# aclike/dynamic_multiview_3d

Measured on AMD Instinct MI355X. Metric: train images/sec, appearance-flow encoder-decoder 128x128x3 (fwd+bwd+Adam), higher is better.
Workload: dtype bf16x3; 1 GPU; appflow_offset: AppearanceFlowModel 128x128x3, batch 64 per GPU, Adam lr 1e-4, random-init weights (reference initialisers); global_batch=64, parallelism=dp1

## Files before the change

### dynamic_multiview_3d_amd/csrc/fc.hip

```cpp
#include "conv_common.h"
#include <algorithm>

namespace mv3d {

struct FcParams {
    const float* X;
    const float* W;
    float* Part;
    int M, R, N, x_ld;
    int w_ld;
    int nsplit, chunks_total;
};

template <bool TRANS, int MT>
__global__ __launch_bounds__(256) void fc_stream_kernel(const FcParams p) {
    constexpr int LDA = 33;
    constexpr int ROWS = 32 * MT;
    __shared__ float As[2][ROWS * LDA];
    const int tid = threadIdx.x;
    const int lane = tid & 63, wave = tid >> 6;
    const int li = lane & 31, lh = lane >> 5;
    const int n0 = blockIdx.x * 128 + wave * 32;
    const int ks = blockIdx.y;
    const int c_begin = (int)((int64_t)p.chunks_total * ks / p.nsplit);
    const int c_end = (int)((int64_t)p.chunks_total * (ks + 1) / p.nsplit);

    f32x16 acc[MT];
#pragma unroll
    for (int m = 0; m < MT; ++m)
#pragma unroll
        for (int r = 0; r < 16; ++r) acc[m][r] = 0.f;

    const int col = n0 + li;
    const int colc = col < p.N ? col : p.N - 1;

    constexpr int A_PASSES = ROWS / 32;
    float4 ra[A_PASSES];
    auto load_a = [&](int chunk) {
        const int r0 = chunk * 32 + (tid & 7) * 4;
        const bool k_ok = r0 + 4 <= p.R;
#pragma unroll
        for (int ps = 0; ps < A_PASSES; ++ps) {
            const int row = ps * 32 + (tid >> 3);
            const bool ok = k_ok && row < p.M;
            const float4 v = *reinterpret_cast<const float4*>(p.X + (int64_t)(ok ? row : 0) * p.x_ld + (ok ? r0 : 0));
            ra[ps] = ok ? v : make_float4(0.f, 0.f, 0.f, 0.f);
        }
    };
    auto store_a = [&](int buf) {
#pragma unroll
        for (int ps = 0; ps < A_PASSES; ++ps) {
            float* d = &As[buf][(ps * 32 + (tid >> 3)) * LDA + (tid & 7) * 4];
            d[0] = ra[ps].x; d[1] = ra[ps].y; d[2] = ra[ps].z; d[3] = ra[ps].w;
        }
    };
    float b0[16], b1[16];
    auto load_b = [&](float (&b)[16], int chunk) {
        const int r0 = chunk * 32 + lh * 16;
        const int rc = (r0 + 16 <= p.R) ? r0 : 0;
        if constexpr (TRANS) {
            const float4* src = reinterpret_cast<const float4*>(p.W + (int64_t)colc * p.w_ld + rc);
#pragma unroll
            for (int j = 0; j < 4; ++j) {
                const float4 v = src[j];
                b[4 * j] = v.x; b[4 * j + 1] = v.y; b[4 * j + 2] = v.z; b[4 * j + 3] = v.w;
            }
        } else {
            const float* src = p.W + (int64_t)rc * p.w_ld + colc;
#pragma unroll
            for (int kp = 0; kp < 16; ++kp) { b[kp] = *src; src += p.w_ld; }
        }
    };

    if (c_begin < c_end) {
        load_a(c_begin);
        load_b(b1, c_begin);
        store_a(0);
        __syncthreads();
        int buf = 0;
        for (int c = c_begin; c < c_end; ++c, buf ^= 1) {
            const bool more = c + 1 < c_end;
#pragma unroll
            for (int kp = 0; kp < 16; ++kp) b0[kp] = b1[kp];
            if (more) { load_a(c + 1); load_b(b1, c + 1); }
            const float* ap = &As[buf][li * LDA + lh * 16];
#pragma unroll
            for (int kp = 0; kp < 16; ++kp)
#pragma unroll
                for (int m = 0; m < MT; ++m)
                    acc[m] = __builtin_amdgcn_mfma_f32_32x32x2f32(ap[m * 32 * LDA + kp], b0[kp], acc[m], 0, 0, 0);
            if (more) store_a(buf ^ 1);
            __syncthreads();
        }
    }
#pragma unroll
    for (int m = 0; m < MT; ++m)
#pragma unroll
        for (int r = 0; r < 16; ++r) {
            const int row = m * 32 + (r & 3) + 8 * (r >> 2) + 4 * lh;
            if (row < p.M && col < p.N) p.Part[((int64_t)ks * p.M + row) * p.N + col] = acc[m][r];
        }
}


typedef __bf16 fbf16x8 __attribute__((ext_vector_type(8)));
typedef __bf16 fbf16x4 __attribute__((ext_vector_type(4)));
typedef short fs16x4 __attribute__((ext_vector_type(4)));

__device__ __forceinline__ void fsplit4(float a, float b, float c, float d, uint2& hi, uint2& lo) {
    fbf16x4 h, l;
    h[0] = (__bf16)a; h[1] = (__bf16)b; h[2] = (__bf16)c; h[3] = (__bf16)d;
    l[0] = (__bf16)(a - (float)h[0]); l[1] = (__bf16)(b - (float)h[1]);
    l[2] = (__bf16)(c - (float)h[2]); l[3] = (__bf16)(d - (float)h[3]);
    hi = __builtin_bit_cast(uint2, h);
    lo = __builtin_bit_cast(uint2, l);
}

template <bool TRANS, int MT>
__global__ __launch_bounds__(256) void fc_stream_b3_kernel(const FcParams p) {
    constexpr int ROWS = 32 * MT;
    constexpr int RSB = 80;
    __shared__ __attribute__((aligned(16))) unsigned char As[2][2][ROWS * RSB];
    const int tid = threadIdx.x;
    const int lane = tid & 63, wave = tid >> 6;
    const int li = lane & 31, lh = lane >> 5;
    const int n0 = blockIdx.x * 128 + wave * 32;
    const int ks = blockIdx.y;
    const int c_begin = (int)((int64_t)p.chunks_total * ks / p.nsplit);
    const int c_end = (int)((int64_t)p.chunks_total * (ks + 1) / p.nsplit);

    f32x16 acc[MT];
#pragma unroll
    for (int m = 0; m < MT; ++m)
#pragma unroll
        for (int r = 0; r < 16; ++r) acc[m][r] = 0.f;

    const int col = n0 + li;
    const int colc = col < p.N ? col : p.N - 1;

    constexpr int A_PASSES = ROWS / 32;
    constexpr int RING = MT <= 2 ? 6 : 4;
    float4 rq[RING][A_PASSES];
    auto load_a = [&](float4 (&ra)[A_PASSES], int chunk) {
        const int r0 = chunk * 32 + (tid & 7) * 4;
        const bool k_ok = r0 + 4 <= p.R;
#pragma unroll
        for (int ps = 0; ps < A_PASSES; ++ps) {
            const int row = ps * 32 + (tid >> 3);
            const bool ok = k_ok && row < p.M;
            const float4 v = *reinterpret_cast<const float4*>(p.X + (int64_t)(ok ? row : 0) * p.x_ld + (ok ? r0 : 0));
            ra[ps] = ok ? v : make_float4(0.f, 0.f, 0.f, 0.f);
        }
    };
    auto store_a = [&](const float4 (&ra)[A_PASSES], int buf) {
#pragma unroll
        for (int ps = 0; ps < A_PASSES; ++ps) {
            uint2 hi, lo;
            fsplit4(ra[ps].x, ra[ps].y, ra[ps].z, ra[ps].w, hi, lo);
            const int off = (ps * 32 + (tid >> 3)) * RSB + (tid & 7) * 8;
            *reinterpret_cast<uint2*>(&As[buf][0][off]) = hi;
            *reinterpret_cast<uint2*>(&As[buf][1][off]) = lo;
        }
    };
    float bq[RING][16];
    auto load_b = [&](float (&b)[16], int chunk) {
        const int r0 = chunk * 32 + lh * 16;
        const int rc = (r0 + 16 <= p.R) ? r0 : 0;
        if constexpr (TRANS) {
            const float4* src = reinterpret_cast<const float4*>(p.W + (int64_t)colc * p.w_ld + rc);
#pragma unroll
            for (int j = 0; j < 4; ++j) {
                const float4 v = src[j];
                b[4 * j] = v.x; b[4 * j + 1] = v.y; b[4 * j + 2] = v.z; b[4 * j + 3] = v.w;
            }
        } else {
            const float* src = p.W + (int64_t)rc * p.w_ld + colc;
#pragma unroll
            for (int kp = 0; kp < 16; ++kp) { b[kp] = *src; src += p.w_ld; }
        }
    };
    auto mma = [&](const float (&b)[16], int buf) {
#pragma unroll
        for (int s2 = 0; s2 < 2; ++s2) {
            uint2 h0, l0, h1, l1;
            fsplit4(b[8 * s2], b[8 * s2 + 1], b[8 * s2 + 2], b[8 * s2 + 3], h0, l0);
            fsplit4(b[8 * s2 + 4], b[8 * s2 + 5], b[8 * s2 + 6], b[8 * s2 + 7], h1, l1);
            const fbf16x8 bh = __builtin_bit_cast(fbf16x8, make_uint4(h0.x, h0.y, h1.x, h1.y));
            const fbf16x8 bl = __builtin_bit_cast(fbf16x8, make_uint4(l0.x, l0.y, l1.x, l1.y));
#pragma unroll
            for (int m = 0; m < MT; ++m) {
                const int off = (m * 32 + li) * RSB + (lh * 16 + 8 * s2) * 2;
                const fbf16x8 ah = __builtin_bit_cast(fbf16x8, *reinterpret_cast<const uint4*>(&As[buf][0][off]));
                const fbf16x8 al = __builtin_bit_cast(fbf16x8, *reinterpret_cast<const uint4*>(&As[buf][1][off]));
                acc[m] = __builtin_amdgcn_mfma_f32_32x32x16_bf16(al, bh, acc[m], 0, 0, 0);
                acc[m] = __builtin_amdgcn_mfma_f32_32x32x16_bf16(ah, bl, acc[m], 0, 0, 0);
                acc[m] = __builtin_amdgcn_mfma_f32_32x32x16_bf16(ah, bh, acc[m], 0, 0, 0);
            }
        }
    };

    if (c_begin < c_end) {
#pragma unroll
        for (int u = 0; u < RING - 1; ++u) {
            const int cu = c_begin + u < c_end ? c_begin + u : c_end - 1;
            load_a(rq[u], cu);
            load_b(bq[u], cu);
        }
        store_a(rq[0], 0);
        __syncthreads();
        int buf = 0;
        constexpr int NCH = 16;
        if (c_end - c_begin == NCH) {
#pragma unroll
            for (int i = 0; i < NCH; ++i) {
                if (i + RING - 1 < NCH) {
                    load_a(rq[(i + RING - 1) % RING], c_begin + i + RING - 1);
                    load_b(bq[(i + RING - 1) % RING], c_begin + i + RING - 1);
                }
                __builtin_amdgcn_sched_barrier(0);
                mma(bq[i % RING], i & 1);
                if (i + 1 < NCH) store_a(rq[(i + 1) % RING], (i + 1) & 1);
                __syncthreads();
            }
        } else
        for (int c = c_begin; c < c_end; c += RING) {
#pragma unroll
            for (int u = 0; u < RING; ++u) {
                const int cc = c + u;
                if (cc < c_end) {
                    const int cn = cc + RING - 1 < c_end ? cc + RING - 1 : c_end - 1;
                    load_a(rq[(u + RING - 1) % RING], cn);
                    load_b(bq[(u + RING - 1) % RING], cn);
                    mma(bq[u], buf);
                    if (cc + 1 < c_end) store_a(rq[(u + 1) % RING], buf ^ 1);
                    __syncthreads();
                    buf ^= 1;
                }
            }
        }
    }
#pragma unroll
    for (int m = 0; m < MT; ++m)
#pragma unroll
        for (int r = 0; r < 16; ++r) {
            const int row = m * 32 + (r & 3) + 8 * (r >> 2) + 4 * lh;
            if (row < p.M && col < p.N) p.Part[((int64_t)ks * p.M + row) * p.N + col] = acc[m][r];
        }
}

struct FcWgradParams {
    const float* X; const float* DY; float* dW; float* db;
    int B, C, K, x_ld, dy_ld;
    int ktiles;
    float* M1; float* V2;
    const float* state;
};

__device__ __forceinline__ void adam_elem(float g, float& pv, float& mv, float& vv, float alpha, float omb1, float omb2, float eps) {
#pragma clang fp contract(off)
    mv += (g - mv) * omb1;
    vv += (g * g - vv) * omb2;
    pv -= (mv * alpha) / (sqrtf(vv) + eps);
}

__global__ __launch_bounds__(256) void fc_wgrad_kernel(const FcWgradParams p) {
    __shared__ __attribute__((aligned(16))) float xs[64 * 128];
    __shared__ __attribute__((aligned(16))) float dys[64 * 128];
    const int tid = threadIdx.x;
    const int lane = tid & 63, wave = tid >> 6;
    const int li = lane & 31, lh = lane >> 5;
    const int kt = blockIdx.x % p.ktiles, ct = blockIdx.x / p.ktiles;
    const int c0 = ct * 128, k0 = kt * 128;
    const int ws = wave >> 1, wt = wave & 1;
    f32x16 acc[2][2];
#pragma unroll
    for (int a = 0; a < 2; ++a)
#pragma unroll
        for (int b = 0; b < 2; ++b)
#pragma unroll
            for (int r = 0; r < 16; ++r) acc[a][b][r] = 0.f;
    float sb[2] = {0.f, 0.f};
    for (int b0 = 0; b0 < p.B; b0 += 64) {
        if (b0) __syncthreads();
        float4 vx[8], vy[8];
#pragma unroll
        for (int j = 0; j < 8; ++j) {
            const int row = b0 + (tid >> 5) + 8 * j;
            const int cx = c0 + (tid & 31) * 4, ky = k0 + (tid & 31) * 4;
            const bool okx = row < p.B && cx + 4 <= p.C, oky = row < p.B && ky + 4 <= p.K;
            const float4 tx = *reinterpret_cast<const float4*>(p.X + (okx ? (int64_t)row * p.x_ld + cx : 0));
            const float4 ty = *reinterpret_cast<const float4*>(p.DY + (oky ? (int64_t)row * p.dy_ld + ky : 0));
            vx[j] = okx ? tx : make_float4(0.f, 0.f, 0.f, 0.f);
            vy[j] = oky ? ty : make_float4(0.f, 0.f, 0.f, 0.f);
        }
#pragma unroll
        for (int j = 0; j < 8; ++j) {
            const int r = (tid >> 5) + 8 * j;
            *reinterpret_cast<float4*>(&xs[r * 128 + (tid & 31) * 4]) = vx[j];
            *reinterpret_cast<float4*>(&dys[r * 128 + (tid & 31) * 4]) = vy[j];
        }
        __syncthreads();
        const float* pa = xs + lh * 128 + ws * 64 + li;
        const float* pb = dys + lh * 128 + wt * 64 + li;
#pragma unroll 4
        for (int bp = 0; bp < 32; ++bp) {
            const float a0 = pa[bp * 256], a1 = pa[bp * 256 + 32];
            const float q0 = pb[bp * 256], q1 = pb[bp * 256 + 32];
            acc[0][0] = __builtin_amdgcn_mfma_f32_32x32x2f32(a0, q0, acc[0][0], 0, 0, 0);
            acc[0][1] = __builtin_amdgcn_mfma_f32_32x32x2f32(a0, q1, acc[0][1], 0, 0, 0);
            acc[1][0] = __builtin_amdgcn_mfma_f32_32x32x2f32(a1, q0, acc[1][0], 0, 0, 0);
            acc[1][1] = __builtin_amdgcn_mfma_f32_32x32x2f32(a1, q1, acc[1][1], 0, 0, 0);
            sb[0] += q0; sb[1] += q1;
        }
    }
#pragma unroll
    for (int s = 0; s < 2; ++s)
#pragma unroll
        for (int t = 0; t < 2; ++t) {
            const int k = k0 + wt * 64 + t * 32 + li;
#pragma unroll
            for (int r = 0; r < 16; ++r) {
                const int c = c0 + ws * 64 + s * 32 + (r & 3) + 8 * (r >> 2) + 4 * lh;
                if (c < p.C && k < p.K) p.dW[(int64_t)c * p.K + k] = acc[s][t][r];
            }
        }
    if (p.db && ct == 0 && ws == 0) {
#pragma unroll
        for (int t = 0; t < 2; ++t) {
            const float v = sb[t] + __shfl_xor(sb[t], 32);
            const int k = k0 + wt * 64 + t * 32 + li;
            if (lh == 0 && k < p.K) p.db[k] = v;
        }
    }
}


__device__ __forceinline__ uint2 ftr_read(const unsigned char* lds_ptr) {
    fs16x4 v = __builtin_amdgcn_ds_read_tr16_b64_v4i16((__attribute__((address_space(3))) fs16x4*)lds_ptr);
    return __builtin_bit_cast(uint2, v);
}

template <int OPT>
__global__ __launch_bounds__(256) void fc_wgrad_b3_kernel(const FcWgradParams p) {
    constexpr int RS = 320;
    __shared__ __attribute__((aligned(16))) unsigned char xs[2][32 * RS];
    __shared__ __attribute__((aligned(16))) unsigned char dys[2][32 * RS];
    __shared__ float bred[8][128];
    const int tid = threadIdx.x;
    const int lane = tid & 63, wave = tid >> 6;
    const int li = lane & 31, lh = lane >> 5;
    const int kt = blockIdx.x % p.ktiles, ct = blockIdx.x / p.ktiles;
    const int c0 = ct * 128, k0 = kt * 128;
    const int ws = wave >> 1, wt = wave & 1;
    const int g16 = (lane >> 4) & 1, q = (lane >> 2) & 3, pp = lane & 3;
    f32x16 acc[2][2];
#pragma unroll
    for (int a = 0; a < 2; ++a)
#pragma unroll
        for (int b = 0; b < 2; ++b)
#pragma unroll
            for (int r = 0; r < 16; ++r) acc[a][b][r] = 0.f;
    float4 bs = make_float4(0.f, 0.f, 0.f, 0.f);
    for (int b0 = 0; b0 < p.B; b0 += 32) {
        if (b0) __syncthreads();
        float4 vx[4], vy[4];
#pragma unroll
        for (int j = 0; j < 4; ++j) {
            const int row = b0 + (tid >> 5) + 8 * j;
            const int cx = c0 + (tid & 31) * 4, ky = k0 + (tid & 31) * 4;
            const bool okx = row < p.B && cx + 4 <= p.C, oky = row < p.B && ky + 4 <= p.K;
            const float4 tx = *reinterpret_cast<const float4*>(p.X + (okx ? (int64_t)row * p.x_ld + cx : 0));
            const float4 ty = *reinterpret_cast<const float4*>(p.DY + (oky ? (int64_t)row * p.dy_ld + ky : 0));
            vx[j] = okx ? tx : make_float4(0.f, 0.f, 0.f, 0.f);
            vy[j] = oky ? ty : make_float4(0.f, 0.f, 0.f, 0.f);
        }
#pragma unroll
        for (int j = 0; j < 4; ++j) {
            const int off = ((tid >> 5) + 8 * j) * RS + (tid & 31) * 8;
            uint2 hi, lo;
            fsplit4(vx[j].x, vx[j].y, vx[j].z, vx[j].w, hi, lo);
            *reinterpret_cast<uint2*>(&xs[0][off]) = hi;
            *reinterpret_cast<uint2*>(&xs[1][off]) = lo;
            fsplit4(vy[j].x, vy[j].y, vy[j].z, vy[j].w, hi, lo);
            *reinterpret_cast<uint2*>(&dys[0][off]) = hi;
            *reinterpret_cast<uint2*>(&dys[1][off]) = lo;
            bs.x += vy[j].x; bs.y += vy[j].y; bs.z += vy[j].z; bs.w += vy[j].w;
        }
        __syncthreads();
#pragma unroll
        for (int s2 = 0; s2 < 2; ++s2) {
            const int row0 = 16 * s2 + 8 * lh + q;
            const int ra0 = row0 * RS + (16 * g16 + 4 * pp) * 2, ra1 = ra0 + 4 * RS;
            fbf16x8 ah[2], al[2], bh[2], bl[2];
#pragma unroll
            for (int t = 0; t < 2; ++t) {
                const int ca = (ws * 64 + t * 32) * 2, cb = (wt * 64 + t * 32) * 2;
                uint2 u0 = ftr_read(&xs[0][ra0 + ca]), u1 = ftr_read(&xs[0][ra1 + ca]);
                ah[t] = __builtin_bit_cast(fbf16x8, make_uint4(u0.x, u0.y, u1.x, u1.y));
                u0 = ftr_read(&xs[1][ra0 + ca]); u1 = ftr_read(&xs[1][ra1 + ca]);
                al[t] = __builtin_bit_cast(fbf16x8, make_uint4(u0.x, u0.y, u1.x, u1.y));
                u0 = ftr_read(&dys[0][ra0 + cb]); u1 = ftr_read(&dys[0][ra1 + cb]);
                bh[t] = __builtin_bit_cast(fbf16x8, make_uint4(u0.x, u0.y, u1.x, u1.y));
                u0 = ftr_read(&dys[1][ra0 + cb]); u1 = ftr_read(&dys[1][ra1 + cb]);
                bl[t] = __builtin_bit_cast(fbf16x8, make_uint4(u0.x, u0.y, u1.x, u1.y));
            }
#pragma unroll
            for (int a = 0; a < 2; ++a)
#pragma unroll
                for (int b = 0; b < 2; ++b) {
                    acc[a][b] = __builtin_amdgcn_mfma_f32_32x32x16_bf16(al[a], bh[b], acc[a][b], 0, 0, 0);
                    acc[a][b] = __builtin_amdgcn_mfma_f32_32x32x16_bf16(ah[a], bl[b], acc[a][b], 0, 0, 0);
                    acc[a][b] = __builtin_amdgcn_mfma_f32_32x32x16_bf16(ah[a], bh[b], acc[a][b], 0, 0, 0);
                }
        }
    }
    float alpha = 0.f, omb1 = 0.f, omb2 = 0.f, eps = 0.f, gscale = 1.f;
    float lr = 0.f, mu = 0.f;
    bool nesterov = false;
    if constexpr (OPT == OPT_MOMENTUM || OPT == OPT_GD) {
        lr = p.state[MV3D_SGD_LR]; mu = p.state[MV3D_SGD_MOMENTUM]; nesterov = p.state[MV3D_SGD_NESTEROV] != 0.f;
        gscale = p.state[MV3D_SGD_GSCALE];
    }
    if constexpr (OPT == OPT_ADAM) {
        const float lr = p.state[0], b1 = p.state[1], b2 = p.state[2], b1p = p.state[4], b2p = p.state[5];
        eps = p.state[3]; gscale = p.state[6];
        {
#pragma clang fp contract(off)
            alpha = lr * sqrtf(1.0f - b2p) / (1.0f - b1p);
            omb1 = 1.0f - b1; omb2 = 1.0f - b2;
        }
    }
#pragma unroll
    for (int s = 0; s < 2; ++s)
#pragma unroll
        for (int t = 0; t < 2; ++t) {
            const int k = k0 + wt * 64 + t * 32 + li;
            if constexpr (OPT == OPT_ADAM) {
                {
                    float pv[16], mv[16], vv[16];
#pragma unroll
                    for (int r = 0; r < 16; ++r) {
                        const int c = c0 + ws * 64 + s * 32 + (r & 3) + 8 * (r >> 2) + 4 * lh;
                        const int64_t idx = (c < p.C && k < p.K) ? (int64_t)c * p.K + k : 0;
                        pv[r] = p.dW[idx]; mv[r] = p.M1[idx]; vv[r] = p.V2[idx];
                    }
#pragma unroll
                    for (int r = 0; r < 16; ++r) adam_elem(acc[s][t][r] * gscale, pv[r], mv[r], vv[r], alpha, omb1, omb2, eps);
#pragma unroll
                    for (int r = 0; r < 16; ++r) {
                        const int c = c0 + ws * 64 + s * 32 + (r & 3) + 8 * (r >> 2) + 4 * lh;
                        if (c < p.C && k < p.K) {
                            const int64_t idx = (int64_t)c * p.K + k;
                            p.dW[idx] = pv[r]; p.M1[idx] = mv[r]; p.V2[idx] = vv[r];
                        }
                    }
                }
            } else if constexpr (OPT == OPT_MOMENTUM || OPT == OPT_GD) {
                float pv[16], av[16];
#pragma unroll
                for (int r = 0; r < 16; ++r) {
                    const int c = c0 + ws * 64 + s * 32 + (r & 3) + 8 * (r >> 2) + 4 * lh;
                    const int64_t idx = (c < p.C && k < p.K) ? (int64_t)c * p.K + k : 0;
                    pv[r] = p.dW[idx];
                    if constexpr (OPT == OPT_MOMENTUM) av[r] = p.M1[idx];
                }
#pragma unroll
                for (int r = 0; r < 16; ++r) {
                    if constexpr (OPT == OPT_MOMENTUM) momentum_elem(acc[s][t][r] * gscale, pv[r], av[r], lr, mu, nesterov);
                    else gd_elem(acc[s][t][r] * gscale, pv[r], lr);
                }
#pragma unroll
                for (int r = 0; r < 16; ++r) {
                    const int c = c0 + ws * 64 + s * 32 + (r & 3) + 8 * (r >> 2) + 4 * lh;
                    if (c < p.C && k < p.K) {
                        const int64_t idx = (int64_t)c * p.K + k;
                        p.dW[idx] = pv[r];
                        if constexpr (OPT == OPT_MOMENTUM) p.M1[idx] = av[r];
                    }
                }
            } else {
#pragma unroll
                for (int r = 0; r < 16; ++r) {
                    const int c = c0 + ws * 64 + s * 32 + (r & 3) + 8 * (r >> 2) + 4 * lh;
                    if (c < p.C && k < p.K) p.dW[(int64_t)c * p.K + k] = acc[s][t][r];
                }
            }
        }
    if (p.db && ct == 0) {
        float* br = &bred[tid >> 5][(tid & 31) * 4];
        br[0] = bs.x; br[1] = bs.y; br[2] = bs.z; br[3] = bs.w;
        __syncthreads();
        if (tid < 128) {
            float t = 0.f;
#pragma unroll
            for (int r = 0; r < 8; ++r) t += bred[r][tid];
            if (k0 + tid < p.K) p.db[k0 + tid] = t;
        }
    }
}

static bool fc_stream_ok(int B, int in, int out, const void* x, int x_ld, const void* W, bool trans) {
    if (B < 1 || B > 128) return false;
    const int R = trans ? out : in;
    if (R < 256 || R % 16 != 0 || x_ld % 4 != 0) return false;
    if ((reinterpret_cast<uintptr_t>(x) & 15) || (reinterpret_cast<uintptr_t>(W) & 15)) return false;
    if (trans && (out % 4 != 0)) return false;
    return !(disabled_paths() & 16);
}

static int fc_target_wgs() {
    static int v = -1;
    if (v < 0) { const char* e = getenv("MV3D_FC_WGS"); v = e ? atoi(e) : 256; }
    return v;
}

size_t fc_stream_ws_bytes(int B, int in, int out, bool trans) {
    const int R = trans ? out : in, N = trans ? in : out;
    const int chunks = cdiv(R, 32);
    int nsplit = std::max(1, std::min(chunks / 4, cdiv(fc_target_wgs(), cdiv(N, 128))));
    return (size_t)nsplit * B * N * sizeof(float);
}

int try_fc_stream(bool trans, int B, int in, int out, const void* x, int x_ld, const void* W, void* y, int y_ld,
                  const mv3d_epilogue* epi, void* ws, size_t wsb, void* stream, const char* who,
                  void (*fill_epi)(IgemmParams&, const mv3d_epilogue*), void (*launch_epi)(const IgemmParams&, int, hipStream_t)) {
    if (!fc_stream_ok(B, in, out, x, x_ld, W, trans)) return 1;
    FcParams p = {};
    p.X = (const float*)x; p.W = (const float*)W; p.Part = (float*)ws;
    p.M = B; p.R = trans ? out : in; p.N = trans ? in : out; p.x_ld = x_ld; p.w_ld = out;
    p.chunks_total = cdiv(p.R, 32);
    p.nsplit = std::max(1, std::min(p.chunks_total / 4, cdiv(fc_target_wgs(), cdiv(p.N, 128))));
    const size_t need = (size_t)p.nsplit * B * p.N * sizeof(float);
    if (!ws || wsb < need) return 1;
    dim3 grid(cdiv(p.N, 128), p.nsplit);
    const int MT = cdiv(B, 32);
    const double flops = 2.0 * B * (double)in * out, bytes = 4.0 * ((double)in * out + (double)B * (in + out));
    const bool b3 = !(disabled_paths() & 4096);
    int rc = dispatch(stream, OpInfo{b3 ? (trans ? "fc_stream_b3<dgrad>" : "fc_stream_b3<fwd>") : (trans ? "fc_stream<dgrad>" : "fc_stream<fwd>"), flops, bytes}, [=](hipStream_t s) {
        if (b3) {
            if (trans) {
                if (MT <= 1) fc_stream_b3_kernel<true, 1><<<grid, 256, 0, s>>>(p);
                else if (MT == 2) fc_stream_b3_kernel<true, 2><<<grid, 256, 0, s>>>(p);
                else fc_stream_b3_kernel<true, 4><<<grid, 256, 0, s>>>(p);
            } else {
                if (MT <= 1) fc_stream_b3_kernel<false, 1><<<grid, 256, 0, s>>>(p);
                else if (MT == 2) fc_stream_b3_kernel<false, 2><<<grid, 256, 0, s>>>(p);
                else fc_stream_b3_kernel<false, 4><<<grid, 256, 0, s>>>(p);
            }
        } else if (trans) {
            if (MT <= 1) fc_stream_kernel<true, 1><<<grid, 256, 0, s>>>(p);
            else if (MT == 2) fc_stream_kernel<true, 2><<<grid, 256, 0, s>>>(p);
            else fc_stream_kernel<true, 4><<<grid, 256, 0, s>>>(p);
        } else {
            if (MT <= 1) fc_stream_kernel<false, 1><<<grid, 256, 0, s>>>(p);
            else if (MT == 2) fc_stream_kernel<false, 2><<<grid, 256, 0, s>>>(p);
            else fc_stream_kernel<false, 4><<<grid, 256, 0, s>>>(p);
        }
        return launched(who);
    });
    if (rc != MV3D_OK) return rc;
    IgemmParams e = {};
    e.N = 1; e.Hc = 1; e.Wc = B; e.Cc = p.N; e.c_ld = y_ld; e.Out = (float*)y; e.Part = (float*)ws; e.ksplit = p.nsplit;
    fill_epi(e, epi);
    const int64_t total = (int64_t)B * p.N;
    const int blocks = (int)std::min<int64_t>(cdiv64(total, 256), 4096);
    return dispatch(stream, OpInfo{"fc_splitk_epilogue", 0.0, (double)total * 4.0 * (p.nsplit + 1)}, [=](hipStream_t s) {
        launch_epi(e, blocks, s);
        return launched("igemm_splitk_epilogue");
    });
}

int try_fc_wgrad(int B, int in, int out, const void* x, int x_ld, const void* dy, int dy_ld, void* dM, void* db, void* stream, const char* who) {
    if (B < 2 || in < 64 || out < 64 || (disabled_paths() & 16)) return 1;
    if (in % 4 || out % 4 || x_ld % 4 || dy_ld % 4 || (reinterpret_cast<uintptr_t>(x) & 15) || (reinterpret_cast<uintptr_t>(dy) & 15)) return 1;
    FcWgradParams p = {(const float*)x, (const float*)dy, (float*)dM, (float*)db, B, in, out, x_ld, dy_ld, cdiv(out, 128), nullptr, nullptr, nullptr};
    const int items = cdiv(in, 128) * p.ktiles;
    const double flops = 2.0 * B * (double)in * out, bytes = 4.0 * ((double)in * out + (double)B * (in + out));
    const bool b3 = !(disabled_paths() & 4096);
    return dispatch(stream, OpInfo{b3 ? "fc_wgrad_b3" : "fc_wgrad", flops, bytes}, [=](hipStream_t s) {
        if (b3) fc_wgrad_b3_kernel<OPT_NONE><<<items, 256, 0, s>>>(p);
        else fc_wgrad_kernel<<<items, 256, 0, s>>>(p);
        return launched(who);
    });
}

int try_fc_wgrad_adam(int B, int in, int out, const void* x, int x_ld, const void* dy, int dy_ld, void* P, void* M1, void* V2, void* db,
                      const void* state, void* stream, const char* who) {
    if (B < 2 || in < 64 || out < 64 || (disabled_paths() & (16 | 4096))) return 1;
    if (in % 4 || out % 4 || x_ld % 4 || dy_ld % 4 || (reinterpret_cast<uintptr_t>(x) & 15) || (reinterpret_cast<uintptr_t>(dy) & 15)) return 1;
    FcWgradParams p = {(const float*)x, (const float*)dy, (float*)P, (float*)db, B, in, out, x_ld, dy_ld, cdiv(out, 128), (float*)M1, (float*)V2, (const float*)state};
    const int items = cdiv(in, 128) * p.ktiles;
    const double flops = 2.0 * B * (double)in * out, bytes = 24.0 * (double)in * out + 4.0 * (double)B * (in + out);
    return dispatch(stream, OpInfo{"fc_wgrad_adam_b3", flops, bytes}, [=](hipStream_t s) {
        fc_wgrad_b3_kernel<OPT_ADAM><<<items, 256, 0, s>>>(p);
        return launched(who);
    });
}

int try_fc_wgrad_sgd(int B, int in, int out, const void* x, int x_ld, const void* dy, int dy_ld, void* P, void* A, void* db,
                     const void* state, void* stream, const char* who) {
    if (B < 2 || in < 64 || out < 64 || (disabled_paths() & (16 | 4096))) return 1;
    if (in % 4 || out % 4 || x_ld % 4 || dy_ld % 4 || (reinterpret_cast<uintptr_t>(x) & 15) || (reinterpret_cast<uintptr_t>(dy) & 15)) return 1;
    FcWgradParams p = {(const float*)x, (const float*)dy, (float*)P, (float*)db, B, in, out, x_ld, dy_ld, cdiv(out, 128), (float*)A, nullptr, (const float*)state};
    const int items = cdiv(in, 128) * p.ktiles;
    const bool mom = A != nullptr;
    const double flops = 2.0 * B * (double)in * out, bytes = (mom ? 16.0 : 8.0) * (double)in * out + 4.0 * (double)B * (in + out);
    return dispatch(stream, OpInfo{mom ? "fc_wgrad_momentum_b3" : "fc_wgrad_sgd_b3", flops, bytes}, [=](hipStream_t s) {
        if (mom) fc_wgrad_b3_kernel<OPT_MOMENTUM><<<items, 256, 0, s>>>(p);
        else fc_wgrad_b3_kernel<OPT_GD><<<items, 256, 0, s>>>(p);
        return launched(who);
    });
}

}
```

Baseline: 38850 images/sec.

## Use buffer loads and a fully unrolled chunked pipeline in bf16x3 FC kernel

Replaces the FC streaming kernel's global pointer loads with AMD buffer-resource loads. Out-of-range rows and chunks now return zero through the hardware bounds check, so the selects and 64-bit address arithmetic go away. The old split between an unrolled 16-chunk path and a generic ring loop becomes a single 18-chunk compile-time-unrolled pipeline that early-exits on partial groups. The ring depth is fixed at 4 for all MT, where MT≤2 previously used 6. The aim is lower address and branch overhead and full unrolling for any split size, at the cost of a shallower prefetch for small batches and a new 2GB size guard.

Result: no change. 39220 images/sec, median of 6 (+0.9%).

```diff
diff --git a/dynamic_multiview_3d_amd/csrc/fc.hip b/dynamic_multiview_3d_amd/csrc/fc.hip
--- a/dynamic_multiview_3d_amd/csrc/fc.hip
+++ b/dynamic_multiview_3d_amd/csrc/fc.hip
@@ -1,5 +1,6 @@
 #include "conv_common.h"
 #include <algorithm>
+#include <utility>
 
 namespace mv3d {
 
@@ -10,6 +11,7 @@
     int M, R, N, x_ld;
     int w_ld;
     int nsplit, chunks_total;
+    int x_bytes, w_bytes;
 };
 
 template <bool TRANS, int MT>
@@ -116,10 +118,15 @@
     lo = __builtin_bit_cast(uint2, l);
 }
 
-template <bool TRANS, int MT>
+template <class F, int... Is>
+__device__ __forceinline__ void fc_chain(F& f, std::integer_sequence<int, Is...>) { (void)(f(std::integral_constant<int, Is>{}) && ...); }
+
+template <bool TRANS, int MT, int RING>
 __global__ __launch_bounds__(256) void fc_stream_b3_kernel(const FcParams p) {
     constexpr int ROWS = 32 * MT;
     constexpr int RSB = 80;
+    constexpr int NCH = 18;
+    constexpr unsigned OOR = 0x7ffffff0u;
     __shared__ __attribute__((aligned(16))) unsigned char As[2][2][ROWS * RSB];
     const int tid = threadIdx.x;
     const int lane = tid & 63, wave = tid >> 6;
@@ -137,20 +144,22 @@
 
     const int col = n0 + li;
     const int colc = col < p.N ? col : p.N - 1;
+    const __amdgpu_buffer_rsrc_t xr = __builtin_amdgcn_make_buffer_rsrc(const_cast<float*>(p.X), 0, p.x_bytes, 0x00020000);
+    const __amdgpu_buffer_rsrc_t wr = __builtin_amdgcn_make_buffer_rsrc(const_cast<float*>(p.W), 0, p.w_bytes, 0x00020000);
 
     constexpr int A_PASSES = ROWS / 32;
-    constexpr int RING = MT <= 2 ? 6 : 4;
+    unsigned va[A_PASSES];
+#pragma unroll
+    for (int ps = 0; ps < A_PASSES; ++ps) {
+        const int row = ps * 32 + (tid >> 3);
+        va[ps] = row < p.M ? ((unsigned)row * (unsigned)p.x_ld + (tid & 7) * 4) * 4u : OOR;
+    }
     float4 rq[RING][A_PASSES];
-    auto load_a = [&](float4 (&ra)[A_PASSES], int chunk) {
-        const int r0 = chunk * 32 + (tid & 7) * 4;
-        const bool k_ok = r0 + 4 <= p.R;
-#pragma unroll
-        for (int ps = 0; ps < A_PASSES; ++ps) {
-            const int row = ps * 32 + (tid >> 3);
-            const bool ok = k_ok && row < p.M;
-            const float4 v = *reinterpret_cast<const float4*>(p.X + (int64_t)(ok ? row : 0) * p.x_ld + (ok ? r0 : 0));
-            ra[ps] = ok ? v : make_float4(0.f, 0.f, 0.f, 0.f);
-        }
+    auto load_a = [&](float4 (&ra)[A_PASSES], int chunk, bool valid) {
+        const bool ok = valid && chunk * 32 + (tid & 7) * 4 + 4 <= p.R;
+#pragma unroll
+        for (int ps = 0; ps < A_PASSES; ++ps)
+            ra[ps] = __builtin_bit_cast(float4, __builtin_amdgcn_raw_buffer_load_b128(xr, ok ? va[ps] : OOR, chunk * 128, 0));
     };
     auto store_a = [&](const float4 (&ra)[A_PASSES], int buf) {
 #pragma unroll
@@ -162,21 +171,21 @@
             *reinterpret_cast<uint2*>(&As[buf][1][off]) = lo;
         }
     };
+    const unsigned vb = TRANS ? ((unsigned)colc * (unsigned)p.w_ld + lh * 16) * 4u : ((unsigned)(lh * 16) * (unsigned)p.w_ld + colc) * 4u;
     float bq[RING][16];
-    auto load_b = [&](float (&b)[16], int chunk) {
-        const int r0 = chunk * 32 + lh * 16;
-        const int rc = (r0 + 16 <= p.R) ? r0 : 0;
+    auto load_b = [&](float (&b)[16], int chunk, bool valid) {
+        const bool ok = valid && chunk * 32 + lh * 16 + 16 <= p.R;
+        const unsigned v = ok ? vb : OOR;
         if constexpr (TRANS) {
-            const float4* src = reinterpret_cast<const float4*>(p.W + (int64_t)colc * p.w_ld + rc);
 #pragma unroll
             for (int j = 0; j < 4; ++j) {
-                const float4 v = src[j];
-                b[4 * j] = v.x; b[4 * j + 1] = v.y; b[4 * j + 2] = v.z; b[4 * j + 3] = v.w;
+                const float4 t = __builtin_bit_cast(float4, __builtin_amdgcn_raw_buffer_load_b128(wr, v + 16 * j, chunk * 128, 0));
+                b[4 * j] = t.x; b[4 * j + 1] = t.y; b[4 * j + 2] = t.z; b[4 * j + 3] = t.w;
             }
         } else {
-            const float* src = p.W + (int64_t)rc * p.w_ld + colc;
-#pragma unroll
-            for (int kp = 0; kp < 16; ++kp) { b[kp] = *src; src += p.w_ld; }
+#pragma unroll
+            for (int kp = 0; kp < 16; ++kp)
+                b[kp] = __uint_as_float(__builtin_amdgcn_raw_buffer_load_b32(wr, v, (chunk * 32 + kp) * p.w_ld * 4, 0));
         }
     };
     auto mma = [&](const float (&b)[16], int buf) {
@@ -199,45 +208,29 @@
         }
     };
 
-    if (c_begin < c_end) {
+    for (int c0 = c_begin; c0 < c_end; c0 += NCH) {
+        const int n = c_end - c0 < NCH ? c_end - c0 : NCH;
 #pragma unroll
         for (int u = 0; u < RING - 1; ++u) {
-            const int cu = c_begin + u < c_end ? c_begin + u : c_end - 1;
-            load_a(rq[u], cu);
-            load_b(bq[u], cu);
+            load_a(rq[u], c0 + u, u < n);
+            load_b(bq[u], c0 + u, u < n);
         }
         store_a(rq[0], 0);
         __syncthreads();
-        int buf = 0;
-        constexpr int NCH = 16;
-        if (c_end - c_begin == NCH) {
-#pragma unroll
-            for (int i = 0; i < NCH; ++i) {
-                if (i + RING - 1 < NCH) {
-                    load_a(rq[(i + RING - 1) % RING], c_begin + i + RING - 1);
-                    load_b(bq[(i + RING - 1) % RING], c_begin + i + RING - 1);
-                }
-                __builtin_amdgcn_sched_barrier(0);
-                mma(bq[i % RING], i & 1);
-                if (i + 1 < NCH) store_a(rq[(i + 1) % RING], (i + 1) & 1);
-                __syncthreads();
-            }
-        } else
-        for (int c = c_begin; c < c_end; c += RING) {
-#pragma unroll
-            for (int u = 0; u < RING; ++u) {
-                const int cc = c + u;
-                if (cc < c_end) {
-                    const int cn = cc + RING - 1 < c_end ? cc + RING - 1 : c_end - 1;
-                    load_a(rq[(u + RING - 1) % RING], cn);
-                    load_b(bq[(u + RING - 1) % RING], cn);
-                    mma(bq[u], buf);
-                    if (cc + 1 < c_end) store_a(rq[(u + 1) % RING], buf ^ 1);
-                    __syncthreads();
-                    buf ^= 1;
-                }
-            }
-        }
+        auto step = [&](auto ic) {
+            constexpr int i = decltype(ic)::value;
+            if (i >= n) return false;
+            if constexpr (i + RING - 1 < NCH) {
+                load_a(rq[(i + RING - 1) % RING], c0 + i + RING - 1, i + RING - 1 < n);
+                load_b(bq[(i + RING - 1) % RING], c0 + i + RING - 1, i + RING - 1 < n);
+            }
+            __builtin_amdgcn_sched_barrier(0);
+            mma(bq[i % RING], i & 1);
+            if constexpr (i + 1 < NCH) store_a(rq[(i + 1) % RING], (i + 1) & 1);
+            __syncthreads();
+            return true;
+        };
+        fc_chain(step, std::make_integer_sequence<int, NCH>{});
     }
 #pragma unroll
     for (int m = 0; m < MT; ++m)
@@ -499,12 +492,14 @@
     }
 }
 
+constexpr int FC_RING = 4;
 static bool fc_stream_ok(int B, int in, int out, const void* x, int x_ld, const void* W, bool trans) {
     if (B < 1 || B > 128) return false;
     const int R = trans ? out : in;
     if (R < 256 || R % 16 != 0 || x_ld % 4 != 0) return false;
     if ((reinterpret_cast<uintptr_t>(x) & 15) || (reinterpret_cast<uintptr_t>(W) & 15)) return false;
     if (trans && (out % 4 != 0)) return false;
+    if ((int64_t)in * out * 4 >= 0x7ffffff0 || ((int64_t)(B - 1) * x_ld + R) * 4 >= 0x7ffffff0) return false;
     return !(disabled_paths() & 16);
 }
 
@@ -528,6 +523,7 @@
     FcParams p = {};
     p.X = (const float*)x; p.W = (const float*)W; p.Part = (float*)ws;
     p.M = B; p.R = trans ? out : in; p.N = trans ? in : out; p.x_ld = x_ld; p.w_ld = out;
+    p.x_bytes = (int)(((int64_t)(B - 1) * x_ld + p.R) * 4); p.w_bytes = (int)((int64_t)in * out * 4);
     p.chunks_total = cdiv(p.R, 32);
     p.nsplit = std::max(1, std::min(p.chunks_total / 4, cdiv(fc_target_wgs(), cdiv(p.N, 128))));
     const size_t need = (size_t)p.nsplit * B * p.N * sizeof(float);
@@ -539,13 +535,13 @@
     int rc = dispatch(stream, OpInfo{b3 ? (trans ? "fc_stream_b3<dgrad>" : "fc_stream_b3<fwd>") : (trans ? "fc_stream<dgrad>" : "fc_stream<fwd>"), flops, bytes}, [=](hipStream_t s) {
         if (b3) {
             if (trans) {
-                if (MT <= 1) fc_stream_b3_kernel<true, 1><<<grid, 256, 0, s>>>(p);
-                else if (MT == 2) fc_stream_b3_kernel<true, 2><<<grid, 256, 0, s>>>(p);
-                else fc_stream_b3_kernel<true, 4><<<grid, 256, 0, s>>>(p);
+                if (MT <= 1) fc_stream_b3_kernel<true, 1, FC_RING><<<grid, 256, 0, s>>>(p);
+                else if (MT == 2) fc_stream_b3_kernel<true, 2, FC_RING><<<grid, 256, 0, s>>>(p);
+                else fc_stream_b3_kernel<true, 4, FC_RING><<<grid, 256, 0, s>>>(p);
             } else {
-                if (MT <= 1) fc_stream_b3_kernel<false, 1><<<grid, 256, 0, s>>>(p);
-                else if (MT == 2) fc_stream_b3_kernel<false, 2><<<grid, 256, 0, s>>>(p);
-                else fc_stream_b3_kernel<false, 4><<<grid, 256, 0, s>>>(p);
+                if (MT <= 1) fc_stream_b3_kernel<false, 1, FC_RING><<<grid, 256, 0, s>>>(p);
+                else if (MT == 2) fc_stream_b3_kernel<false, 2, FC_RING><<<grid, 256, 0, s>>>(p);
+                else fc_stream_b3_kernel<false, 4, FC_RING><<<grid, 256, 0, s>>>(p);
             }
         } else if (trans) {
             if (MT <= 1) fc_stream_kernel<true, 1><<<grid, 256, 0, s>>>(p);
```
